# VikParuchuri/surya

Hardware: AMD Instinct MI355X
Metric: text-lines/sec recognised (whole node) (higher is better)
Workload: dtype bf16; 1 GPU; RecognitionPredictor device loop, 256 ragged 64x{128..512} crops/GPU, batch 256, max_tokens=48, REC-FULL synthetic weights (conditioned recipe, seed 0), tiles resident in HBM; parallelism=1 GPU, weights=conditioned

## Files before the change

surya_amd/csrc/attn_mfma.h:

```cpp
#pragma once
#include "common.h"
#include "kernels.h"

namespace sa {

typedef short s16x4 __attribute__((ext_vector_type(4)));

template <typename T, int D>
__global__ __launch_bounds__(128) void attn_mfma_kernel(const T* __restrict__ q, const T* __restrict__ k,
                                                        const T* __restrict__ v, T* __restrict__ out, AttnSegs sg,
                                                        long q_row, long q_head, long k_row, long k_head, long o_row, long o_head,
                                                        int group, int causal, float scale) {
    static_assert(D % 16 == 0 && D <= 128, "head dim");
    static_assert(sizeof(T) == 2, "16-bit storage types");
    constexpr int KC = 64;
    constexpr int PK = D + 8;
    constexpr int NKK = D / 16;
    constexpr int NDB = (D + 31) / 32;
    constexpr int CPR = D / 8;
    __shared__ __attribute__((aligned(16))) T ks[(KC + 1) * PK];
    __shared__ __attribute__((aligned(16))) T vs[(KC + 1) * PK];

    const int tile = blockIdx.x, head = blockIdx.y, kvh = head / group;
    const int seg = sg.tile_seg[tile], q0 = sg.tile_q0[tile], L = sg.seg_len[seg];
    const int tid = threadIdx.x, lane = tid & 63, wave = tid >> 6;
    const int ql = lane & 31, h = lane >> 5;
    const int qi = q0 + wave * 32 + ql;

    u32x4 qf[NKK];
    {
        const T* qp = q + sg.q_off[seg] + (long)min(qi, L - 1) * q_row + (long)head * q_head + h * 8;
#pragma unroll
        for (int kk = 0; kk < NKK; ++kk) qf[kk] = *reinterpret_cast<const u32x4*>(qp + kk * 16);
    }
    f32x16 oacc[NDB];
#pragma unroll
    for (int db = 0; db < NDB; ++db)
#pragma unroll
        for (int r = 0; r < 16; ++r) oacc[db][r] = 0.f;
    float mrun = -INFINITY, lrun = 0.f;
    const float sl2 = scale * 1.44269504088896340736f;

    const int kend = causal ? min(L, q0 + 64) : L;
    const T* kbase = k + sg.k_off[seg] + (long)kvh * k_head;
    const T* vbase = v + sg.v_off[seg] + (long)kvh * k_head;
    const int tr_off = ((lane & 15) >> 2) * PK + ((lane >> 4) & 1) * 16 + (lane & 3) * 4 + h * 4 * PK;

    constexpr int NST = KC * CPR / 128;
    static_assert(KC * CPR % 128 == 0, "staging split");
    u32x4 kreg[NST], vreg[NST];
    auto fetch = [&](int kc) {
        const int nk = min(KC, kend - kc);
#pragma unroll
// ... 48 lines not shown
        mrun = mnew;
        float psum = 0.f;
#pragma unroll
        for (int kb = 0; kb < 2; ++kb)
#pragma unroll
            for (int r = 0; r < 16; ++r) {
                const float pv = exp2f((sacc[kb][r] - mnew) * sl2);
                sacc[kb][r] = pv;
                psum += pv;
            }
        lrun = lrun * alpha + psum;
#pragma unroll
        for (int db = 0; db < NDB; ++db)
#pragma unroll
            for (int r = 0; r < 16; ++r) oacc[db][r] *= alpha;

#pragma unroll
        for (int t = 0; t < 4; ++t) {
            const int kb = t >> 1, o8 = (t & 1) * 8;
            u32x4 pf;
            pf[0] = H16<T>::pk(sacc[kb][o8 + 0], sacc[kb][o8 + 1]);
            pf[1] = H16<T>::pk(sacc[kb][o8 + 2], sacc[kb][o8 + 3]);
            pf[2] = H16<T>::pk(sacc[kb][o8 + 4], sacc[kb][o8 + 5]);
            pf[3] = H16<T>::pk(sacc[kb][o8 + 6], sacc[kb][o8 + 7]);
#pragma unroll
            for (int db = 0; db < NDB; ++db) {
                const T* vp = vs + t * 16 * PK + db * 32 + tr_off;
                const s16x4 lo = __builtin_amdgcn_ds_read_tr16_b64_v4i16((__attribute__((address_space(3))) s16x4*)(vp));
                const s16x4 hi = __builtin_amdgcn_ds_read_tr16_b64_v4i16((__attribute__((address_space(3))) s16x4*)(vp + 8 * PK));
                typedef short s16x8 __attribute__((ext_vector_type(8)));
                const s16x8 vf = __builtin_shufflevector(lo, hi, 0, 1, 2, 3, 4, 5, 6, 7);
                oacc[db] = H16<T>::mfma(vf, pf, oacc[db]);
            }
        }
        __syncthreads();
    }

    const float ltot = lrun + __shfl_xor(lrun, 32, 64);
    if (qi < L) {
        const float inv = 1.0f / ltot;
        T* op = out + sg.o_off[seg] + (long)qi * o_row + (long)head * o_head;
#pragma unroll
        for (int db = 0; db < NDB; ++db)
#pragma unroll
            for (int g = 0; g < 4; ++g) {
                const int d0 = db * 32 + g * 8 + h * 4;
                if (d0 < D) store4(op + d0, oacc[db][4 * g] * inv, oacc[db][4 * g + 1] * inv, oacc[db][4 * g + 2] * inv,
                                   oacc[db][4 * g + 3] * inv);
            }
    }
}

template <typename T>
int launch_attn(int D, const T* q, const T* k, const T* v, T* o, const AttnSegs& sg, int n_tiles, int heads, long q_row, long q_head,
                long k_row, long k_head, long o_row, long o_head, int group, int causal, float scale, hipStream_t s) {
    if (n_tiles <= 0) return SA_OK;
    auto go = [&](auto kern, int threads) {
        hipLaunchKernelGGL(kern, dim3(n_tiles, heads), dim3(threads), 0, s, q, k, v, o, sg, q_row, q_head, k_row, k_head, o_row, o_head, group,
                           causal, scale);
        return (int)hipGetLastError();
    };
    if constexpr (sizeof(T) == 2) {
        if (D == 32) return go(attn_mfma_kernel<T, 32>, 128);
        if (D == 64) return go(attn_mfma_kernel<T, 64>, 128);
        if (D == 80) return go(attn_mfma_kernel<T, 80>, 128);
        if (D == 128) return go(attn_mfma_kernel<T, 128>, 128);
    } else {
        static_assert(std::is_same<T, float>::value, "the VALU kernel is the fp32 reference-mode path only");
        if (D == 32) return go(attn_valu_kernel<T, 32>, 256);
        if (D == 64) return go(attn_valu_kernel<T, 64>, 256);
        if (D == 80) return go(attn_valu_kernel<T, 80>, 256);
        if (D == 128) return go(attn_valu_kernel<T, 128>, 256);
    }
    return SA_ERR_UNSUPPORTED;
}

}
```

surya_amd/csrc/common.h:

```cpp
#pragma once
#include <hip/hip_runtime.h>
#include <cstdlib>
#include <stdint.h>
#include <stdio.h>
#include <type_traits>

#include "../../include/surya_amd.h"

namespace sa {

typedef unsigned short bf16_t;
typedef __attribute__((ext_vector_type(4))) float f32x4;
typedef __attribute__((ext_vector_type(16))) float f32x16;
typedef __attribute__((ext_vector_type(8))) __bf16 bf16x8;
typedef unsigned int u32x4 __attribute__((ext_vector_type(4)));


#define SA_HIP(expr)                                                                                   \
    do {                                                                                               \
        hipError_t _e = (expr);                                                                        \
        if (_e != hipSuccess) {                                                                        \
            fprintf(stderr, "[surya_amd] %s:%d %s -> %s\n", __FILE__, __LINE__, #expr, hipGetErrorString(_e)); \
            return (int)_e;                                                                            \
        }                                                                                              \
// ... 208 lines not shown
    } else {
        return gelu_erf_f(x);
    }
}
__device__ __forceinline__ float gelu_tanh_f(float x) { return 0.5f * x * (1.0f + tanhf(0.7978845608028654f * (x + 0.044715f * x * x * x))); }
__device__ __forceinline__ float sigmoid_f(float x) { return 1.0f / (1.0f + __expf(-x)); }
__device__ __forceinline__ float hardswish_f(float x) {
    float t;
    asm("v_fma_f32 %0, %1, %2, 0.5 clamp" : "=v"(t) : "v"(x), "s"(1.0f / 6.0f));
    return x * t;
}
typedef float f32x2_hs __attribute__((ext_vector_type(2)));
__device__ __forceinline__ f32x2_hs hardswish_pk(f32x2_hs x) {
    f32x2_hs t;
    const f32x2_hs c = {1.0f / 6.0f, 1.0f / 6.0f};
    asm("v_pk_fma_f32 %0, %1, %2, 0.5 op_sel_hi:[1,0,0] clamp" : "=v"(t) : "v"(x), "s"(c));
    return x * t;
}

struct Tuning {
    int graph = 0;
    int split_target = 256;
    int split_min_kt = 4;
    int split_max = 8;
    int bigtile = 3;
    int bigtile_any = 0;
    int big_m_split = -1;
    int big_m_gateup = -1;
    int mx_big_m_split = -1;
    int mx_big_m_gateup = -1;
    int gateup_ring = 2;
    int dring = 1;
    int dring_min_kt = 0;
    int conv_persist = 3;
    int dwconv_pipe = 2;
    int conv_lean = 1;
    int bigtile_ratio_pct = 0;
    int bigtile_min_k = 0;
    int glds = 2;
    int dattn = 4;
    int rnorm = 2;
    int ghead = 2;
    int fuse_embed = 1;
    int kvprefetch = 0;
    int lmhead = 1;
    int dattn_db = 0;
    int lay_ln = 1;
    int det_head_blk = 1;
    int det_fuse = 1023;
    int det_up4 = 1;
    int fmb_chunk = 64;
    int persist = 1;
    int ocrerr_cls_only = 1;
};
inline Tuning& tuning() { static Tuning t; return t; }
inline int& tuning_epoch() { static int e = 0; return e; }

inline void poison_arena(void* p, size_t bytes) {
    static const bool on = [] { const char* e = getenv("SURYA_AMD_POISON"); return e && e[0] == '1'; }();
    if (on) { (void)hipMemset(p, 0xFF, bytes); (void)hipDeviceSynchronize(); }
}

struct AttrOnce {
    size_t granted[64] = {};
    template <typename F> void ensure(F kern, size_t lds) {
        int dev = 0;
        (void)hipGetDevice(&dev);
        size_t& g = granted[dev & 63];
        if (lds > g || g == 0) {
            (void)hipFuncSetAttribute(reinterpret_cast<const void*>(kern), hipFuncAttributeMaxDynamicSharedMemorySize, (int)lds);
            g = lds > g ? lds : g;
            if (g == 0) g = 1;
        }
    }
};

constexpr int SA_ALT_NONE = 0x7fffffff;
__device__ __forceinline__ bool alt_after(float v, int c, float pv, int pc) { return (v < pv) | ((v == pv) & (c > pc)); }
__device__ __forceinline__ bool alt_before(float v, int c, float bv, int bc) { return (v > bv) | ((v == bv) & (c < bc)); }
__device__ __forceinline__ float2 alt_next(const float2* cand, int n, float pv, int pc) {
    float cb = -INFINITY;
    int ci = SA_ALT_NONE;
    for (int k = 0; k < n; ++k) {
        const float v = cand[k].x;
        const int cc = __float_as_int(cand[k].y);
        const bool take = (v > -INFINITY) & alt_after(v, cc, pv, pc) & alt_before(v, cc, cb, ci);
        cb = take ? v : cb;
        ci = take ? cc : ci;
    }
    return make_float2(cb, __int_as_float(ci));
}

static inline int cdiv(int a, int b) { return (a + b - 1) / b; }
static inline long cdivl(long a, long b) { return (a + b - 1) / b; }

}
```

surya_amd/csrc/rec_engine.h:

```cpp
#pragma once
#include <algorithm>
#include <cstdlib>
#include <cstring>
#include <initializer_list>
#include <map>
#include <memory>
#include <set>
#include <vector>

#include "../../include/surya_amd.h"
#include "gemm.h"
#include "gemm_mx.h"
#include "kernels.h"
#include "decode_attn.h"
#include "decode_attn_kv8.h"
#include "attn_mfma.h"
#include "beam.h"
#include "lexicon.h"
#include "boost.h"

namespace sa {

struct Stager {
    char* host = nullptr;
// ... 564 lines not shown
                    return rc;
                if ((rc = rmsnorm(ex, He, WE(l, SA_RE_NORM2), eh, He, nullptr, Pi, He, c.enc_eps, s))) return rc;
                if ((rc = gemm<EPI_SWIGLU>(eh, He, WE(l, SA_RE_GU_W), He, emlp, c.enc_inter_pad, WE(l, SA_RE_GU_B), nullptr, 0,
                                           Pi, 2 * c.enc_inter_pad, He, s))) return rc;
                if ((rc = gemm<EPI_RESIDUAL>(emlp, c.enc_inter_pad, WE(l, SA_RE_DOWN_W), c.enc_inter_pad, ex, He,
                                             WE(l, SA_RE_DOWN_B), ex, He, Pi, He, c.enc_inter_pad, s))) return rc;
            }
            if ((rc = rmsnorm(ex, He, W(SA_RW_MERGER_LN), eh, He, nullptr, Pi, He, 1e-6f, s))) return rc;
            const int Mg = Pi / unit, Hm = He * unit;
            if ((rc = gemm<EPI_GELU>(eh, Hm, W(SA_RW_FC1_W), Hm, emh, Hm, W(SA_RW_FC1_B), nullptr, 0, Mg, Hm, Hm, s))) return rc;
            if ((rc = gemm<EPI_BIAS>(emh, Hm, W(SA_RW_FC2_W), Hm, emerged, c.enc_out_hidden, W(SA_RW_FC2_B), nullptr, 0, Mg,
                                     c.enc_out_hidden, Hm, s))) return rc;
            if ((rc = launch_scatter_image<T>(emerged, W(SA_RW_IMG_H), W(SA_RW_IMG_W), d_dst, d_hidx, d_widx, dst, Mg, c.dec_hidden, s))) return rc;
            patch_base += P;
            tok_base += P / unit;
            i0 = i1;
        }
        return SA_OK;
    }

    int encode_only(const float* tiles, const int32_t* grid_hw, int n, void* out, hipStream_t s) override {
        if (c.enc_out_hidden != c.dec_hidden) return SA_ERR_SHAPE;
        long ntok = 0;
        for (int i = 0; i < n; ++i) ntok += (long)grid_hw[2 * i] * grid_hw[2 * i + 1] / (c.merge * c.merge);
        std::vector<int> ident(ntok);
        for (long i = 0; i < ntok; ++i) ident[i] = (int)i;
        return encode(tiles, grid_hw, n, ident, reinterpret_cast<T*>(out), s);
    }

    int encode_ahead(const float* tiles, const int32_t* grid_hw, int n, hipStream_t s) override {
        if (c.enc_out_hidden != c.dec_hidden) return SA_ERR_SHAPE;
        if (n == 0) {
            ahead_consumed = ahead_tokens = 0;
            return SA_OK;
        }
        if (n < 0 || !tiles || !grid_hw) return SA_ERR_ARG;
        if (ahead_consumed != ahead_tokens) return SA_ERR_STATE;
        long ntok = 0;
        for (int i = 0; i < n; ++i) ntok += (long)grid_hw[2 * i] * grid_hw[2 * i + 1] / (c.merge * c.merge);
        if (ntok > std::max(c.max_prefill_tokens, c.max_slots)) return SA_ERR_SHAPE;
        std::vector<int> ident(ntok);
        for (long i = 0; i < ntok; ++i) ident[i] = (int)i;
        SA_HIP(hipEventRecord(ev_ahead_in, s));
        SA_HIP(hipStreamWaitEvent(estream, ev_ahead_in, 0));
        if (ahead_free_recorded) SA_HIP(hipStreamWaitEvent(estream, ev_ahead_free, 0));
        int rc = encode(tiles, grid_hw, n, ident, emb_ahead, estream, st_enc);
        if (rc) return rc;
        SA_HIP(hipEventRecord(ev_ahead_done, estream));
        ahead_tokens = ntok;
        ahead_consumed = 0;
        return SA_OK;
    }

    int decoder_layers_prefill(int M, const int* d_tok_slot, const int* d_tok_pos, const AttnSegs* sg, int n_tiles, hipStream_t s) {
        const int Hd = c.dec_hidden, nq = c.dec_heads, nkv = c.dec_kv_heads, d = c.dec_head_dim, I = c.dec_inter;
        const int qkv_d = (nq + 2 * nkv) * d;
        const float scale = 1.0f / sqrtf((float)d);
        const size_t layer_kv = (size_t)c.max_slots * nkv * c.max_kv_len * d;
        const float* inv_freq = reinterpret_cast<const float*>(w[SA_RW_DEC_INVFREQ]);
        int rc;
        for (int l = 0; l < c.dec_layers; ++l) {
            T* kc = kcache + l * layer_kv;
            T* vc = vcache + l * layer_kv;
            if ((rc = rmsnorm(dx, Hd, WD(l, SA_RD_LN1), dh, Hd, nullptr, M, Hd, c.dec_eps, s))) return rc;
            if ((rc = gemm<EPI_BIAS>(dh, Hd, WD(l, SA_RD_QKV_W), Hd, dqkv, qkv_d, WD(l, SA_RD_QKV_B), nullptr, 0, M, qkv_d, Hd, s)))
                return rc;
            if ((rc = launch_rope_kv_append<T>(dqkv, d_tok_slot, d_tok_pos, rope_cs, kc, vc, M, nq, nkv, d, c.max_kv_len, s))) return rc;
            if constexpr (std::is_same<T, bf16_t>::value) {
                if (kv8) {
                    const size_t l8 = (size_t)c.max_slots * nkv, T8 = tmax8();
                    if ((rc = launch_kv8_quant_rows(d, kc, vc, d_tok_slot, d_tok_pos, M, k8c + l * l8 * c.max_kv_len * d, v8tc + l * l8 * d * T8,
                                                    ksc8 + l * l8 * T8, vsc8 + l * l8 * T8, nkv, c.max_kv_len, s))) return rc;
                }
            }
            if ((rc = launch_attn<T>(d, dqkv, kc, vc, dattn, *sg, n_tiles, nq, qkv_d, d, d, (long)c.max_kv_len * d, (long)nq * d, d,
                                     nq / nkv, 1, scale, s))) return rc;
            if ((rc = gemm<EPI_RESIDUAL>(dattn, (long)nq * d, WD(l, SA_RD_O_W), (long)nq * d, dx, Hd, nullptr, dx, Hd, M, Hd, nq * d,
                                         s))) return rc;
            if ((rc = rmsnorm(dx, Hd, WD(l, SA_RD_LN2), dh, Hd, nullptr, M, Hd, c.dec_eps, s))) return rc;
            if ((rc = gemm<EPI_SWIGLU>(dh, Hd, WD(l, SA_RD_GU_W), Hd, dmlp, I, nullptr, nullptr, 0, M, 2 * I, Hd, s))) return rc;
            if ((rc = gemm<EPI_RESIDUAL>(dmlp, I, WD(l, SA_RD_DOWN_W), I, dx, Hd, nullptr, dx, Hd, M, Hd, I, s))) return rc;
        }
        return SA_OK;
    }

    struct Half { int r0, M; float* part; hipStream_t s; };

    int splitk_gemm(const T* X, long ldx, const T* Wt, long ldw, int M, int N, int K, float* part_, int* S, hipStream_t s) {
        GemmArgs<T, T> a{X, ldx, Wt, ldw, nullptr, 0, nullptr, nullptr, 0, M, N, K, 1, part_};
        int rc = launch_gemm_splitk<T>(a, s);
        *S = a.splitk;
        return rc;
    }
    int reduce_residual_norm(int S, int M, const float* part_, T* x, const T* wnorm, T* y, hipStream_t s, uint8_t* y8 = nullptr,
                             uint8_t* sy = nullptr, const T* pf_cache = nullptr, const Half* h = nullptr) {
        KvPrefetch pf;
        if (pf_cache && h && tuning().kvprefetch && (c.dec_head_dim * sizeof(T)) % 16 == 0) {
            pf.base = reinterpret_cast<const unsigned char*>(pf_cache);
            pf.slots = active_dev + h->r0; pf.lens = row_len + h->r0;
            pf.head_stride = (long)c.max_kv_len * c.dec_head_dim * sizeof(T);
            pf.slot_stride = pf.head_stride * c.dec_kv_heads;
            pf.heads = c.dec_kv_heads; pf.row_bytes = c.dec_head_dim * (int)sizeof(T); pf.max_rows = c.max_kv_len;
        }
        return launch_reduce_norm<T>(part_, S, M, x, wnorm, y, c.dec_hidden, c.dec_eps, y8, sy, c.max_slots, pf, s);
    }
    int splitk_gemm_mx(const uint8_t* X, const uint8_t* SX, long ldx, const uint8_t* Wq, const uint8_t* SW, int M, int N, int K,
                       float* part_, int* S, hipStream_t s) {
        MxArgs a{X, ldx, SX, Wq, (long)K, SW, M, N, K, (long)c.max_slots, (long)N};
        a.part = part_;
        int rc = launch_gemm_mx_splitk(a, s);
        *S = a.splitk;
        return rc;
    }

    void drop_graphs() {
        for (auto& kv : graphs) (void)hipGraphExecDestroy(kv.second);
        graphs.clear(); seen_keys.clear();
    }
    int set_kv_fp8(int on) override {
        if constexpr (!std::is_same<T, bf16_t>::value) return on ? SA_ERR_UNSUPPORTED : SA_OK;
        if (on && excluded(M_KV8)) return SA_ERR_STATE;
        if ((on != 0) != kv8) drop_graphs();
        if (!on) { kv8 = false; return SA_OK; }
        const int d = c.dec_head_dim;
        if (d != 128 && d != 64 && d != 32) return SA_ERR_UNSUPPORTED;
        if (c.dec_heads / c.dec_kv_heads > 8) return SA_ERR_UNSUPPORTED;
        if (!kv8_arena.dev) {
            const size_t rows = (size_t)c.dec_layers * c.max_slots * c.dec_kv_heads, T8 = tmax8();
            Carve cv;
// ... 610 lines not shown
        int rc, S = 1;
        const bool q8 = mx();
        const int A = nq * d;
        uint8_t *hh8 = nullptr, *shh = nullptr, *at8 = nullptr, *sat = nullptr, *ml8 = nullptr, *sml = nullptr;
        if (q8) {
            hh8 = dh8 + (size_t)h.r0 * Hd; shh = sdh + (size_t)h.r0 * 4;
            at8 = dattn8 + (size_t)h.r0 * A; sat = sattn + (size_t)h.r0 * 4;
            ml8 = dmlp8 + (size_t)h.r0 * I; sml = smlp + (size_t)h.r0 * 4;
        }
        rc = -1;
        if constexpr (MX_OK) {
            if (q8) rc = splitk_gemm_mx(hh8, shh, Hd, MXW(l, SA_MX_QKV_W), MXW(l, SA_MX_QKV_S), M, qkv_d, Hd, h.part, &S, s);
        }
        if (!q8) rc = splitk_gemm(hh, Hd, WD(l, SA_RD_QKV_W), Hd, M, qkv_d, Hd, h.part, &S, s);
        if (rc) return rc;
        bool launched = false;
        if constexpr (std::is_same<T, bf16_t>::value) {
            if (kv8) {
                const size_t l8 = (size_t)c.max_slots * nkv, T8 = tmax8();
                DecodeAttnKv8Args a{h.part, S, WD(l, SA_RD_QKV_B), at, k8c + l * l8 * c.max_kv_len * d, v8tc + l * l8 * d * T8, ksc8 + l * l8 * T8,
                                    vsc8 + l * l8 * T8, act, rl, rope_cs, M, nq, nkv, d, c.max_kv_len, scale, at8, sat, c.max_slots};
                if ((rc = launch_decode_attn_kv8(a, s))) return rc;
                launched = true;
            }
        }
        if (!launched) {
            DecodeAttnArgs<T> a{h.part, S, WD(l, SA_RD_QKV_B), at, kc, vc, act, rl, rope_cs, M, nq, nkv, d, c.max_kv_len, scale, ctx_bound, at8, sat,
                                c.max_slots};
            if ((rc = launch_decode_attn<T>(a, s))) return rc;
        }
        const bool last = (l + 1 == c.dec_layers);
        const T* wnext = last ? W(SA_RW_DEC_NORM) : WD(l + 1, SA_RD_LN1);
        T* ynext = last ? dlast + (size_t)h.r0 * Hd : hh;
        if constexpr (MX_OK) if (q8) {
            if ((rc = splitk_gemm_mx(at8, sat, A, MXW(l, SA_MX_O_W), MXW(l, SA_MX_O_S), M, Hd, A, h.part, &S, s))) return rc;
            if ((rc = reduce_residual_norm(S, M, h.part, x, WD(l, SA_RD_LN2), hh, s, hh8, shh))) return rc;
            MxArgs g{hh8, Hd, shh, MXW(l, SA_MX_GU_W), Hd, MXW(l, SA_MX_GU_S), M, 2 * I, Hd, (long)c.max_slots, (long)2 * I};
            g.Q = ml8; g.ldq = I; g.SQ = sml; g.sq_rows = c.max_slots;
            if ((rc = launch_gemm_mx<MX_EPI_SWIGLU>(g, s))) return rc;
            if ((rc = splitk_gemm_mx(ml8, sml, I, MXW(l, SA_MX_DOWN_W), MXW(l, SA_MX_DOWN_S), M, Hd, I, h.part, &S, s))) return rc;
            return reduce_residual_norm(S, M, h.part, x, wnext, ynext, s, last ? dlast8 + (size_t)h.r0 * Hd : hh8,
                                        last ? slast + (size_t)h.r0 * 4 : shh);
        }
        const bool warm = !last && !kv8;
        const T* v_next = warm ? vcache + (size_t)(l + 1) * layer_kv : nullptr;
        const T* k_next = warm ? kcache + (size_t)(l + 1) * layer_kv : nullptr;
        if ((rc = splitk_gemm(at, (long)nq * d, WD(l, SA_RD_O_W), (long)nq * d, M, Hd, nq * d, h.part, &S, s))) return rc;
        if ((rc = reduce_residual_norm(S, M, h.part, x, WD(l, SA_RD_LN2), hh, s, nullptr, nullptr, v_next, &h))) return rc;
        if ((rc = gemm<EPI_SWIGLU>(hh, Hd, WD(l, SA_RD_GU_W), Hd, ml, I, nullptr, nullptr, 0, M, 2 * I, Hd, s))) return rc;
        if ((rc = splitk_gemm(ml, I, WD(l, SA_RD_DOWN_W), I, M, Hd, I, h.part, &S, s))) return rc;
        return reduce_residual_norm(S, M, h.part, x, wnext, ynext, s, nullptr, nullptr, k_next, &h);
    }

    int heads(int rows, const int* d_last_row, const int* d_row_slot, int step, int len_inc, bool normed, hipStream_t s, bool fuse_next = false) {
        const int Hd = c.dec_hidden;
        int rc;
        T* last = dlast;
        float4* am = amax;
        if (!normed && (rc = rmsnorm(dx, Hd, W(SA_RW_DEC_NORM), last, Hd, d_last_row, rows, Hd, c.dec_eps, s))) return rc;
        int bn_used = 0;
        auto lm_head = [&](auto& a, auto&& launch) -> int {
            a.amax = am;
            if (forcing) {
                a.forced = forced_cols(d_row_slot);
            } else {
                if (n_token_masks > 0) a.tmask = token_mask(d_row_slot);
                if (topk()) a.alt = alt_part;
            }
            const int rc_ =forcing ? launch(a, HeadEpi<0>{}) : topk() ? launch(a, HeadEpi<1>{}) : n_token_masks > 0 ? launch(a, HeadEpi<2>{}) : launch(a, HeadEpi<3>{});
            bn_used = a.bn_used;
            if (rc_ || bst_states == 0) return rc_;
            a.amax = amax_b;
            a.tmask = TokenMask{};
            const int rc_b = launch(a, HeadEpi<3>{});
            return rc_b ? rc_b : a.bn_used != bn_used ? (int)SA_ERR_STATE : (int)SA_OK;
        };
        if (mx() && normed) {
            if constexpr (std::is_same<T, bf16_t>::value) {
                static constexpr int EPIS[4] = {MX_EPI_FORCED, MX_EPI_TOPK, MX_EPI_ARGMAX_MASK, MX_EPI_ARGMAX};
                MxArgs a{dlast8, Hd, slast, MXG(SA_MX_LM_W), Hd, MXG(SA_MX_LM_S), rows, c.vocab, Hd, (long)c.max_slots, (long)c.vocab};
                a.bias = W(SA_RW_LM_B);
                if ((rc = lm_head(a, [&](MxArgs& a_, auto e) { return launch_gemm_mx<EPIS[decltype(e)::value]>(a_, s); }))) return rc;
            }
        } else {
            static constexpr int EPIS[4] = {EPI_FORCED, EPI_TOPK, EPI_ARGMAX_MASK, EPI_ARGMAX};
            GemmArgs<T, float> a{last, Hd, W(SA_RW_LM_W), Hd, logits, c.vocab, W(SA_RW_LM_B), nullptr, 0, rows, c.vocab, Hd};
            if ((rc = lm_head(a, [&](GemmArgs<T, float>& a_, auto e) { return launch_gemm<T, float, EPIS[decltype(e)::value]>(a_, s); }))) return rc;
        }
        const int tiles_n = cdiv(c.vocab, bn_used);
        const size_t so = (size_t)step * c.max_slots;
        last_rows = rows;
        last_heads_mx = mx() && normed;
        float2* bt = topk() ? best_tot : nullptr;
        ForcedHead fh;
        if (forcing) fh = ForcedHead{forced_table, forced_cursor, flogit, SA_MAX_FORCED_TOKENS, greedy_token + so, greedy_prob + so, forced_logprob + so};
        auto combine = [&]() -> int {
            if ((rc = (int)hipGetLastError()) || !topk()) return rc;
            hipLaunchKernelGGL(topk_combine_kernel, dim3(rows), dim3(SA_ALT_THREADS), 0, s, alt_part, tiles_n, d_row_slot, bt,
                               alt_token + so * SA_MAX_ALTERNATIVES, alt_prob + so * SA_MAX_ALTERNATIVES);
            return (int)hipGetLastError();
        };
        const bool fz = fuse_next;
        HeadArgs<T> ha{reinterpret_cast<const float4*>(am), tiles_n, rows, last, Hd, W(SA_RW_BBOX_W), W(SA_RW_BBOX_B), d_row_slot, c.eos_token_id,
                       c.pad_token_id, (float)c.bbox_size, out_token + so, out_score + so, out_bbox + so * 6, next_token, kv_len, len_inc};
        ha.table = fz ? W(SA_RW_TOK_EMBED) : (const T*)nullptr;
        ha.wnorm = WD(0, SA_RD_LN1); ha.x = dx; ha.y = dh; ha.row_len = row_len; ha.Tmax = c.max_kv_len; ha.eps = c.dec_eps;
        ha.y8 = (fz && mx()) ? dh8 : (uint8_t*)nullptr; ha.sy = (fz && mx()) ? sdh : (uint8_t*)nullptr; ha.srows = c.max_slots;
        ha.best_tot = bt; ha.fh = fh;
        if (pat_states > 0)
            ha.ph = PatternHead{pat_tok_class, pat_next_state, pat_state_mask, SA_MAX_PATTERN_CLASSES, c.vocab, slot_state, slot_mask};
        if (bst_states > 0) {
            BoostHeadArgs<T> bh{ha, reinterpret_cast<const float4*>(amax_b), slot_bst_beta, plain_token + so, plain_prob + so};
// ... 24 lines not shown
            for (int t = 0; t < L; ++t) {
                const int id = input_ids[a + t];
                if (id < 0 || id >= c.vocab) return SA_ERR_ARG;
                const bool img = (id == c.image_token_id);
                ids[a + t] = img ? -1 : id;
                if (img) img_pos.push_back(a + t);
                tok_slot[a + t] = slot_ids[i]; tok_pos[a + t] = t;
            }
            sg.seg_len.push_back(L);
            sg.q_off.push_back((long)a * (nq + 2 * nkv) * d);
            sg.k_off.push_back((long)slot_ids[i] * nkv * c.max_kv_len * d);
            sg.v_off.push_back((long)slot_ids[i] * nkv * c.max_kv_len * d);
            sg.o_off.push_back((long)a * nq * d);
            sg.add_tiles(i, L);
        }
        long ntok = 0;
        for (int i = 0; i < n_images; ++i) ntok += (long)grid_hw[2 * i] * grid_hw[2 * i + 1] / (c.merge * c.merge);
        if ((long)img_pos.size() != ntok) return SA_ERR_SHAPE;
        int rc;
        st_small.begin();
        const int* d_slots = st_small.put(slot_ids, n_seqs);
        const int* d_lens = st_small.put(lens);
        const int* d_last = st_small.put(last_row);
        if (!d_last) return SA_ERR_NOMEM;
        if ((rc = st_small.flush(s))) return rc;
        {
            st.begin();
            const int* d_ids = st.put(ids);
            if (!d_ids) return SA_ERR_NOMEM;
            if ((rc = st.flush(s))) return rc;
            if ((rc = launch_embed_tokens<T>(W(SA_RW_TOK_EMBED), d_ids, dx, Ttot, c.dec_hidden, s))) return rc;
        }
        if (n_images > 0 && tiles) {
            if ((rc = encode(tiles, grid_hw, n_images, img_pos, dx, s))) return rc;
        } else if (n_images > 0) {
            if (ahead_consumed + ntok > ahead_tokens) return SA_ERR_STATE;
            st.begin();
            const int* d_img = st.put(img_pos);
            if (!d_img) return SA_ERR_NOMEM;
            if ((rc = st.flush(s))) return rc;
            SA_HIP(hipStreamWaitEvent(s, ev_ahead_done, 0));
            if ((rc = launch_scatter_rows<T>(emb_ahead + ahead_consumed * c.dec_hidden, d_img, dx, (int)ntok, c.dec_hidden, s))) return rc;
            ahead_consumed += ntok;
            SA_HIP(hipEventRecord(ev_ahead_free, s));
            ahead_free_recorded = true;
        }
        st.begin();
        const int* d_tok_slot = st.put(tok_slot);
        const int* d_tok_pos = st.put(tok_pos);
        AttnSegs d_sg = stage_segs(st, sg);
        if (!d_sg.o_off) return SA_ERR_NOMEM;
        if ((rc = st.flush(s))) return rc;
        hipLaunchKernelGGL(set_slot_state_kernel, dim3(cdiv(n_seqs, 256)), dim3(256), 0, s, d_slots, d_lens, kv_len, n_seqs);
        if ((rc = decoder_layers_prefill(Ttot, d_tok_slot, d_tok_pos, &d_sg, (int)sg.tile_seg.size(), s))) return rc;
        if ((rc = heads(n_seqs, d_last, d_slots, 0, 0, false, s)) || beam == 0) return rc;
        return beam_step(d_slots, 1, n_seqs, 0, 1, s);
    }

    int set_active(const int32_t* slots, int n, hipStream_t s) override {
        if (n < 0 || n > c.max_slots) return SA_ERR_ARG;
        n_active = n;
        for (int i = 0; i < n; ++i)
            if (slots[i] < 0 || slots[i] >= c.max_slots) return SA_ERR_ARG;
        if (beam > 0) {
            if (n % beam) return SA_ERR_ARG;
            for (int i = 0; i < n; ++i) {
                const int lead = slots[i - i % beam];
                if (lead % beam || slots[i] != lead + i % beam || (i >= beam && i % beam == 0 && lead <= slots[i - beam])) return SA_ERR_ARG;
            }
        }
        h_active.assign(slots, slots + n);
        if (n == 0) return SA_OK;
        st_small.begin();
        const int* d = st_small.put(slots, n);
        if (!d) return SA_ERR_NOMEM;
        int rc = st_small.flush(s);
        if (rc) return rc;
        SA_HIP(hipMemcpyAsync(active_dev, d, n * sizeof(int), hipMemcpyDeviceToDevice, s));
        return SA_OK;
    }

    bool can_fuse_embed() const {
        return tuning().fuse_embed && head2_ok() && c.dec_hidden <= 2 * 4 * SA_HEAD_THREADS && cdiv(c.vocab, 320) <= 4 * SA_HEAD_THREADS &&
               cdiv(c.vocab, 64) <= 4 * SA_HEAD_THREADS;
    }
    int decode_eager(int M, int n_steps, int step0, hipStream_t s) {
        int rc;
        const Half h{0, M, part, s};
        const bool fuse = can_fuse_embed() && beam == 0;
        if (h_len.size() < (size_t)c.max_slots) h_len.resize(c.max_slots, 0);
        for (int step = 0; step < n_steps; ++step) {
            ctx_bound = 0;
            for (int a : h_active) {
                ctx_bound = std::max(ctx_bound, h_len[a] + 1);
                h_len[a] = std::min(h_len[a] + 1, c.max_kv_len);
            }
            if ((step == 0 || !fuse) && (rc = decode_embed(h))) return rc;
            for (int l = 0; l < c.dec_layers; ++l)
                if ((rc = decode_layer(l, h))) return rc;
            if ((rc = heads(M, nullptr, active_dev, step0 + step, 1, true, s, fuse && step + 1 < n_steps))) return rc;
            if (beam > 0 && (rc = beam_step(active_dev, beam, M / beam, step0 + step, 0, s))) return rc;
        }
        return SA_OK;
    }

    int decode(int n_steps, hipStream_t s) override { return decode_steps(n_steps, 0, s); }

    int decode_async(int n_steps, int ring, hipStream_t s) override {
// ... 93 lines not shown
```

surya_amd/csrc/rec_model.hip:

```cpp
#include "rec_engine.h"
#include "rec_ops.h"
#include "rec_prep.h"

namespace sa {

template <int D, int MAXG>
static int decode_attn_flash(const DecodeAttnArgs<bf16_t>& a, hipStream_t s) {
    const Tuning& t = tuning();
    if (t.dattn == 3) return decode_attn_as<decode_attn_flash_kernel<D, MAXG>>(a, decode_attn_flash_lds<D, MAXG>(), s, a.out8, a.sout, a.srows);
    if (t.dattn_db == 1 || (t.dattn_db == 0 && !t.graph && a.ctx_bound > 128 && a.rows * a.nkv <= 256))
        return decode_attn_as<decode_attn_flash2_kernel<D, MAXG, true>>(a, decode_attn_flash2_lds<D, MAXG, true>(), s, a.out8, a.sout, a.srows);
    return decode_attn_as<decode_attn_flash2_kernel<D, MAXG, false>>(a, decode_attn_flash2_lds<D, MAXG, false>(), s, a.out8, a.sout, a.srows);
}
template <typename T>
int launch_decode_attn(const DecodeAttnArgs<T>& a, hipStream_t s) {
    const int G = a.nq / a.nkv, d = a.d;
    if constexpr (std::is_same<T, bf16_t>::value) {
        if (d == 128 && G <= 5) return decode_attn_flash<128, 5>(a, s);
        if (d == 128 && G <= 8) return decode_attn_flash<128, 8>(a, s);
        if (d == 64 && G <= 8) return decode_attn_flash<64, 8>(a, s);
        if (d == 32 && G <= 8) return decode_attn_flash<32, 8>(a, s);
    }
    if (a.out8) return SA_ERR_UNSUPPORTED;
    if (d == 128 && G <= 5) return decode_attn_as<decode_attn_mfma_kernel<T, 128, 5>>(a, decode_attn_mfma_lds<T, 128, 5>(), s);
// ... 502 lines not shown
    if (!X || !W || !part || !splitk) return SA_ERR_ARG;
    GemmArgs<bf16_t, bf16_t> a{reinterpret_cast<const bf16_t*>(X), ldx, reinterpret_cast<const bf16_t*>(W), ldw, nullptr, 0, nullptr, nullptr, 0, M, N, K, 1, part};
    const int rc = launch_gemm_splitk<bf16_t>(a, (hipStream_t)stream);
    *splitk = a.splitk;
    return rc;
}

int surya_op_gemm_mx(int mode, const uint8_t* X, const uint8_t* SX, const uint8_t* W, const uint8_t* SW, int M, int N, int K,
                     float* C, int* splitk, uint8_t* q_out, uint8_t* sq_out, void* stream) {
    if (!X || !SX || !W || !SW) return SA_ERR_ARG;
    MxArgs a{X, (long)K, SX, W, (long)K, SW, M, N, K, (long)M, (long)N};
    hipStream_t s = (hipStream_t)stream;
    if (mode == 0) {
        if (!C) return SA_ERR_ARG;
        a.C = C; a.ldc = N;
        return launch_gemm_mx<MX_EPI_F32>(a, s);
    }
    if (mode == 1) {
        if (!C || !splitk) return SA_ERR_ARG;
        a.part = C;
        int rc = launch_gemm_mx_splitk(a, s);
        *splitk = a.splitk;
        return rc;
    }
    if (mode == 2) {
        if (!q_out || !sq_out) return SA_ERR_ARG;
        a.Q = q_out; a.ldq = N / 2; a.SQ = sq_out; a.sq_rows = M;
        return launch_gemm_mx<MX_EPI_SWIGLU>(a, s);
    }
    return SA_ERR_ARG;
}

int surya_rec_preprocess(const uint8_t* pages, const void* lines, int n_lines, uint8_t* mask_arena, float* mid_arena, float* tiles,
                         int patch_size, int merge_size, float pad_value, const float* mean, const float* std, int any_poly,
                         int max_stage1_width, int pixel_stride, void* stream) {
    if (!pages || !lines || !tiles || !mean || !std || n_lines < 0 || patch_size <= 0 || merge_size <= 0) return SA_ERR_ARG;
    if (pixel_stride != 3 && pixel_stride != 4) return SA_ERR_ARG;
    sa::prep::PrepArgs p;
    p.pages = pages; p.lines = reinterpret_cast<const sa::prep::LineDesc*>(lines); p.n_lines = n_lines;
    p.mask = mask_arena; p.mid = mid_arena; p.tiles = tiles; p.ps = patch_size; p.merge = merge_size; p.pad = pad_value;
    for (int i = 0; i < 3; ++i) { p.mean[i] = mean[i]; p.std[i] = std[i]; }
    p.max_mid_w = max_stage1_width;
    p.pix = pixel_stride;
    return sa::prep::prep_run(p, any_poly, max_stage1_width > 0, (hipStream_t)stream);
}

int surya_set_tuning(const char* key, int value) {
    if (!key) return SA_ERR_ARG;
    Tuning& t = tuning();
    struct { const char* k; int* v; } tab[] = {
        {"graph", &t.graph}, {"split_target", &t.split_target}, {"split_min_kt", &t.split_min_kt}, {"split_max", &t.split_max},
        {"bigtile", &t.bigtile}, {"bigtile_any", &t.bigtile_any}, {"conv_lean", &t.conv_lean}, {"conv_persist", &t.conv_persist}, {"dwconv_pipe", &t.dwconv_pipe}, {"bigtile_ratio_pct", &t.bigtile_ratio_pct}, {"gateup_ring", &t.gateup_ring}, {"dring", &t.dring}, {"dring_min_kt", &t.dring_min_kt}, {"big_m_split", &t.big_m_split}, {"big_m_gateup", &t.big_m_gateup}, {"mx_big_m_split", &t.mx_big_m_split}, {"mx_big_m_gateup", &t.mx_big_m_gateup}, {"glds", &t.glds}, {"bigtile_min_k", &t.bigtile_min_k}, {"dattn", &t.dattn}, {"rnorm", &t.rnorm},
        {"ghead", &t.ghead}, {"fuse_embed", &t.fuse_embed}, {"persist", &t.persist}, {"lmhead", &t.lmhead}, {"kvprefetch", &t.kvprefetch},
        {"dattn_db", &t.dattn_db}, {"lay_ln", &t.lay_ln}, {"det_head_blk", &t.det_head_blk}, {"det_fuse", &t.det_fuse}, {"det_up4", &t.det_up4}, {"fmb_chunk", &t.fmb_chunk}, {"ocrerr_cls_only", &t.ocrerr_cls_only}};
    for (auto& e : tab)
        if (!strcmp(e.k, key)) {
            if (*e.v != value) ++tuning_epoch();
            *e.v = value;
            return SA_OK;
        }
    return SA_ERR_ARG;
}

int surya_gemm_ring_status(int reset) {
    const int a = sa::ring_error(reset != 0), b = sa::rec_f16_ring_error(reset != 0);
    return a ? a : b;
}

int surya_prof_enable(int on) {
    GemmProfiler& pf = gemm_profiler();
    if (on) pf.start(); else pf.enabled = false;
    return SA_OK;
}

__global__ void prof_null_kernel() {}

int surya_prof_event_overhead(void* stream, double* ms) {
    if (!ms) return SA_ERR_ARG;
    hipStream_t s = (hipStream_t)stream;
    constexpr int N = 201;
    hipEvent_t ev[2 * N];
    for (auto& e : ev) SA_HIP(hipEventCreate(&e));
    for (int i = 0; i < 32; ++i) hipLaunchKernelGGL(prof_null_kernel, dim3(1), dim3(64), 0, s);
    for (int i = 0; i < N; ++i) {
        SA_HIP(hipEventRecord(ev[2 * i], s));
        hipLaunchKernelGGL(prof_null_kernel, dim3(1), dim3(64), 0, s);
        SA_HIP(hipEventRecord(ev[2 * i + 1], s));
    }
    SA_HIP(hipStreamSynchronize(s));
    std::vector<float> t(N);
    for (int i = 0; i < N; ++i) SA_HIP(hipEventElapsedTime(&t[i], ev[2 * i], ev[2 * i + 1]));
    for (auto& e : ev) (void)hipEventDestroy(e);
    std::sort(t.begin(), t.end());
    *ms = t[N / 2];
    return SA_OK;
}

int surya_prof_read2(int max_cfg, int* launches, double* ms, double* flops, double* bytes, double* slab_bytes) {
    GemmProfiler& pf = gemm_profiler();
    if (!launches || !ms || !flops || !bytes || max_cfg < GemmProfiler::NCFG) return SA_ERR_ARG;
    SA_HIP(hipDeviceSynchronize());
    const int ncfg = std::min(max_cfg, (int)GemmProfiler::NCFG_ALL);
    for (int c = 0; c < ncfg; ++c) { launches[c] = 0; ms[c] = flops[c] = bytes[c] = 0.0; if (slab_bytes) slab_bytes[c] = 0.0; }
    for (int i = 0; i < pf.n; ++i) {
        const int c = pf.cfg_of[i];
        if (c >= ncfg) continue;
        float t = 0.f;
// ... 109 lines not shown
```

Measured before the change: 3150 lines/s.

## Add persistent 4-head vision attention kernel and trim last prefill layer to final rows

After: 3189 lines/s, median of 6. +1.2%, better.

```diff
diff --git a/surya_amd/csrc/attn_mfma.h b/surya_amd/csrc/attn_mfma.h
--- a/surya_amd/csrc/attn_mfma.h
+++ b/surya_amd/csrc/attn_mfma.h
@@ -1,4 +1,6 @@
 #pragma once
+#include <algorithm>
+
 #include "common.h"
 #include "kernels.h"
 
@@ -153,6 +155,190 @@
 }
 
 template <typename T>
+__global__ __launch_bounds__(512) void attn_lines_kernel(const T* __restrict__ q, const T* __restrict__ k, const T* __restrict__ v,
+                                                         T* __restrict__ out, AttnSegs sg, long q_row, long k_row, long o_row, int n_tiles,
+                                                         int n_groups, float scale) {
+    static_assert(sizeof(T) == 2, "16-bit storage types");
+    constexpr int D = 80, HG = 4, KC = 64, PK = D + 8, NKK = D / 16, NDB = (D + 31) / 32, CPR = D / 8;
+    constexpr int RUN = HG * CPR;
+    constexpr int HB = (KC + 1) * PK;
+    extern __shared__ __attribute__((aligned(16))) unsigned char attn_lines_lds[];
+    T* const ks_all = reinterpret_cast<T*>(attn_lines_lds);
+    T* const vs_all = ks_all + HG * HB;
+
+    const int tid = threadIdx.x, lane = tid & 63, wave = tid >> 6;
+    const int hs = wave >> 1, ql = lane & 31, h = lane >> 5;
+    const T* const ks = ks_all + hs * HB;
+    const T* const vs = vs_all + hs * HB;
+    const float sl2 = scale * 1.44269504088896340736f;
+    const int tr_off = ((lane & 15) >> 2) * PK + ((lane >> 4) & 1) * 16 + (lane & 3) * 4 + h * 4 * PK;
+
+    struct Item { int qi, L; const T *qp, *kb, *vb; T* op; };
+    auto item = [&](int w) {
+        const int tile = w / n_groups, hg = w % n_groups;
+        const int seg = sg.tile_seg[tile];
+        Item it;
+        it.L = sg.seg_len[seg];
+        it.qi = sg.tile_q0[tile] + (wave & 1) * 32 + ql;
+        it.qp = q + sg.q_off[seg] + (long)min(it.qi, it.L - 1) * q_row + (long)(hg * HG + hs) * D + h * 8;
+        it.kb = k + sg.k_off[seg] + (long)hg * (HG * D);
+        it.vb = v + sg.v_off[seg] + (long)hg * (HG * D);
+        it.op = out + sg.o_off[seg] + (long)it.qi * o_row + (long)(hg * HG + hs) * D;
+        return it;
+    };
+
+    constexpr int NST = KC * RUN / 512;
+    static_assert(KC * RUN % 512 == 0, "staging split");
+    u32x4 qf[NKK], kreg[NST], vreg[NST];
+    auto fetch_q = [&](const Item& it) {
+#pragma unroll
+        for (int kk = 0; kk < NKK; ++kk) qf[kk] = *reinterpret_cast<const u32x4*>(it.qp + kk * 16);
+    };
+    auto fetch = [&](const T* base, u32x4* reg, int kc, int kend) {
+        const int nk = min(KC, kend - kc);
+#pragma unroll
+        for (int it = 0; it < NST; ++it) {
+            const int c = tid + it * 512, r = min(c / RUN, nk - 1), p = c % RUN;
+            reg[it] = *reinterpret_cast<const u32x4*>(base + (long)(kc + r) * k_row + p * 8);
+        }
+    };
+    auto stage = [&](T* img, const u32x4* reg, int nk) {
+#pragma unroll
+        for (int it = 0; it < NST; ++it) {
+            const int c = tid + it * 512, r = c / RUN, p = c % RUN;
+            const u32x4 z = {0u, 0u, 0u, 0u};
+            *reinterpret_cast<u32x4*>(img + (p / CPR) * HB + r * PK + (p % CPR) * 8) = r < nk ? reg[it] : z;
+        }
+    };
+    const int n_work = n_tiles * n_groups;
+    int w = blockIdx.x;
+    Item cur = item(w);
+    fetch_q(cur);
+    fetch(cur.kb, kreg, 0, cur.L);
+    fetch(cur.vb, vreg, 0, cur.L);
+    for (; w < n_work; w += gridDim.x) {
+        const bool has_next = w + (int)gridDim.x < n_work;
+        const Item nxt = item(has_next ? w + (int)gridDim.x : w);
+        const int kend = cur.L;
+        f32x16 oacc[NDB];
+#pragma unroll
+        for (int db = 0; db < NDB; ++db)
+#pragma unroll
+            for (int r = 0; r < 16; ++r) oacc[db][r] = 0.f;
+        float mrun = -INFINITY, lrun = 0.f;
+        for (int kc = 0; kc < kend; kc += KC) {
+            const int nk = min(KC, kend - kc);
+            const bool last = kc + KC >= kend;
+            stage(ks_all, kreg, nk);
+            stage(vs_all, vreg, nk);
+            __syncthreads();
+            if (!last) {
+                fetch(cur.kb, kreg, kc + KC, kend);
+                fetch(cur.vb, vreg, kc + KC, kend);
+            } else if (has_next) {
+                fetch(nxt.kb, kreg, 0, nxt.L);
+                fetch(nxt.vb, vreg, 0, nxt.L);
+            }
+
+            f32x16 sacc[2];
+#pragma unroll
+            for (int kb = 0; kb < 2; ++kb) {
+#pragma unroll
+                for (int r = 0; r < 16; ++r) sacc[kb][r] = 0.f;
+                const T* kp = ks + (kb * 32 + ql) * PK + h * 8;
+#pragma unroll
+                for (int kk = 0; kk < NKK; ++kk) {
+                    const u32x4 kf = *reinterpret_cast<const u32x4*>(kp + kk * 16);
+                    sacc[kb] = H16<T>::mfma(kf, qf[kk], sacc[kb]);
+                }
+            }
+            if (last && has_next) fetch_q(nxt);
+            float bm = -INFINITY;
+#pragma unroll
+            for (int kb = 0; kb < 2; ++kb)
+#pragma unroll
+                for (int g = 0; g < 4; ++g)
+#pragma unroll
+                    for (int r = 0; r < 4; ++r) {
+                        const int j = kb * 32 + g * 8 + h * 4 + r;
+                        const float sv = (j < nk) ? sacc[kb][4 * g + r] : -INFINITY;
+                        sacc[kb][4 * g + r] = sv;
+                        bm = fmaxf(bm, sv);
+                    }
+            bm = fmaxf(bm, __shfl_xor(bm, 32, 64));
+            const float mnew = fmaxf(mrun, bm);
+            const float alpha = exp2f((mrun - mnew) * sl2);
+            mrun = mnew;
+            float psum = 0.f;
+#pragma unroll
+            for (int kb = 0; kb < 2; ++kb)
+#pragma unroll
+                for (int r = 0; r < 16; ++r) {
+                    const float pv = exp2f((sacc[kb][r] - mnew) * sl2);
+                    sacc[kb][r] = pv;
+                    psum += pv;
+                }
+            lrun = lrun * alpha + psum;
+#pragma unroll
+            for (int db = 0; db < NDB; ++db)
+#pragma unroll
+                for (int r = 0; r < 16; ++r) oacc[db][r] *= alpha;
+
+#pragma unroll
+            for (int t = 0; t < 4; ++t) {
+                const int kb = t >> 1, o8 = (t & 1) * 8;
+                u32x4 pf;
+                pf[0] = H16<T>::pk(sacc[kb][o8 + 0], sacc[kb][o8 + 1]);
+                pf[1] = H16<T>::pk(sacc[kb][o8 + 2], sacc[kb][o8 + 3]);
+                pf[2] = H16<T>::pk(sacc[kb][o8 + 4], sacc[kb][o8 + 5]);
+                pf[3] = H16<T>::pk(sacc[kb][o8 + 6], sacc[kb][o8 + 7]);
+#pragma unroll
+                for (int db = 0; db < NDB; ++db) {
+                    const T* vp = vs + t * 16 * PK + db * 32 + tr_off;
+                    const s16x4 lo = __builtin_amdgcn_ds_read_tr16_b64_v4i16((__attribute__((address_space(3))) s16x4*)(vp));
+                    const s16x4 hi = __builtin_amdgcn_ds_read_tr16_b64_v4i16((__attribute__((address_space(3))) s16x4*)(vp + 8 * PK));
+                    typedef short s16x8 __attribute__((ext_vector_type(8)));
+                    const s16x8 vf = __builtin_shufflevector(lo, hi, 0, 1, 2, 3, 4, 5, 6, 7);
+                    oacc[db] = H16<T>::mfma(vf, pf, oacc[db]);
+                }
+            }
+            __syncthreads();
+        }
+
+        const float ltot = lrun + __shfl_xor(lrun, 32, 64);
+        if (cur.qi < cur.L) {
+            const float inv = 1.0f / ltot;
+#pragma unroll
+            for (int db = 0; db < NDB; ++db)
+#pragma unroll
+                for (int g = 0; g < 4; ++g) {
+                    const int d0 = db * 32 + g * 8 + h * 4;
+                    if (d0 < D) store4(cur.op + d0, oacc[db][4 * g] * inv, oacc[db][4 * g + 1] * inv, oacc[db][4 * g + 2] * inv,
+                                       oacc[db][4 * g + 3] * inv);
+                }
+        }
+        cur = nxt;
+    }
+}
+
+template <typename T>
+int launch_attn_lines(const T* q, const T* k, const T* v, T* o, const AttnSegs& sg, int n_tiles, int heads, long q_row, long k_row, long o_row,
+                      float scale, hipStream_t s) {
+    constexpr size_t lds = (size_t)2 * 4 * 65 * 88 * sizeof(T);
+    static AttrOnce attr;
+    attr.ensure(attn_lines_kernel<T>, lds);
+    static int n_cu_of[64] = {};
+    int dev = 0;
+    (void)hipGetDevice(&dev);
+    int& n_cu = n_cu_of[dev & 63];
+    if (!n_cu && (hipDeviceGetAttribute(&n_cu, hipDeviceAttributeMultiprocessorCount, dev) != hipSuccess || n_cu <= 0)) n_cu = 256;
+    const long n_work = (long)n_tiles * (heads / 4);
+    hipLaunchKernelGGL(attn_lines_kernel<T>, dim3((unsigned)std::min<long>(n_work, n_cu)), dim3(512), lds, s, q, k, v, o, sg, q_row, k_row,
+                       o_row, n_tiles, heads / 4, scale);
+    return (int)hipGetLastError();
+}
+
+template <typename T>
 int launch_attn(int D, const T* q, const T* k, const T* v, T* o, const AttnSegs& sg, int n_tiles, int heads, long q_row, long q_head,
                 long k_row, long k_head, long o_row, long o_head, int group, int causal, float scale, hipStream_t s) {
     if (n_tiles <= 0) return SA_OK;
@@ -162,6 +348,11 @@
         return (int)hipGetLastError();
     };
     if constexpr (sizeof(T) == 2) {
+        if (D == 80 && tuning().vattn && heads % 4 == 0 && group == 1 && !causal && q_head == D && k_head == D && o_head == D && q_row == k_row &&
+            q_row % 64 == 0 && (reinterpret_cast<uintptr_t>(k) - reinterpret_cast<uintptr_t>(q)) % 128 == 0 &&
+            (reinterpret_cast<uintptr_t>(v) - reinterpret_cast<uintptr_t>(q)) % 128 == 0) {
+            return launch_attn_lines<T>(q, k, v, o, sg, n_tiles, heads, q_row, k_row, o_row, scale, s);
+        }
         if (D == 32) return go(attn_mfma_kernel<T, 32>, 128);
         if (D == 64) return go(attn_mfma_kernel<T, 64>, 128);
         if (D == 80) return go(attn_mfma_kernel<T, 80>, 128);
diff --git a/surya_amd/csrc/common.h b/surya_amd/csrc/common.h
--- a/surya_amd/csrc/common.h
+++ b/surya_amd/csrc/common.h
@@ -284,6 +284,8 @@
     int fmb_chunk = 64;
     int persist = 1;
     int ocrerr_cls_only = 1;
+    int vattn = 1;
+    int prefill_trim = 1;
 };
 inline Tuning& tuning() { static Tuning t; return t; }
 inline int& tuning_epoch() { static int e = 0; return e; }
diff --git a/surya_amd/csrc/rec_engine.h b/surya_amd/csrc/rec_engine.h
--- a/surya_amd/csrc/rec_engine.h
+++ b/surya_amd/csrc/rec_engine.h
@@ -640,7 +640,9 @@
         return SA_OK;
     }
 
-    int decoder_layers_prefill(int M, const int* d_tok_slot, const int* d_tok_pos, const AttnSegs* sg, int n_tiles, hipStream_t s) {
+    int decoder_layers_prefill(int M, const int* d_tok_slot, const int* d_tok_pos, const AttnSegs* sg, int n_tiles, const int* d_last_row,
+                               int n_seqs, const T** x_last, hipStream_t s) {
+        *x_last = nullptr;
         const int Hd = c.dec_hidden, nq = c.dec_heads, nkv = c.dec_kv_heads, d = c.dec_head_dim, I = c.dec_inter;
         const int qkv_d = (nq + 2 * nkv) * d;
         const float scale = 1.0f / sqrtf((float)d);
@@ -663,6 +665,18 @@
             }
             if ((rc = launch_attn<T>(d, dqkv, kc, vc, dattn, *sg, n_tiles, nq, qkv_d, d, d, (long)c.max_kv_len * d, (long)nq * d, d,
                                      nq / nkv, 1, scale, s))) return rc;
+            if (l == c.dec_layers - 1 && tuning().prefill_trim && n_seqs < M) {
+                T *ca = dqkv, *cx = dh, *ch = dx;
+                if ((rc = launch_embed_tokens<T>(dattn, d_last_row, ca, n_seqs, nq * d, s))) return rc;
+                if ((rc = launch_embed_tokens<T>(dx, d_last_row, cx, n_seqs, Hd, s))) return rc;
+                if ((rc = gemm<EPI_RESIDUAL>(ca, (long)nq * d, WD(l, SA_RD_O_W), (long)nq * d, cx, Hd, nullptr, cx, Hd, n_seqs, Hd, nq * d,
+                                             s))) return rc;
+                if ((rc = rmsnorm(cx, Hd, WD(l, SA_RD_LN2), ch, Hd, nullptr, n_seqs, Hd, c.dec_eps, s))) return rc;
+                if ((rc = gemm<EPI_SWIGLU>(ch, Hd, WD(l, SA_RD_GU_W), Hd, dmlp, I, nullptr, nullptr, 0, n_seqs, 2 * I, Hd, s))) return rc;
+                if ((rc = gemm<EPI_RESIDUAL>(dmlp, I, WD(l, SA_RD_DOWN_W), I, cx, Hd, nullptr, cx, Hd, n_seqs, Hd, I, s))) return rc;
+                *x_last = cx;
+                return SA_OK;
+            }
             if ((rc = gemm<EPI_RESIDUAL>(dattn, (long)nq * d, WD(l, SA_RD_O_W), (long)nq * d, dx, Hd, nullptr, dx, Hd, M, Hd, nq * d,
                                          s))) return rc;
             if ((rc = rmsnorm(dx, Hd, WD(l, SA_RD_LN2), dh, Hd, nullptr, M, Hd, c.dec_eps, s))) return rc;
@@ -1379,12 +1393,13 @@
         return reduce_residual_norm(S, M, h.part, x, wnext, ynext, s, nullptr, nullptr, k_next, &h);
     }
 
-    int heads(int rows, const int* d_last_row, const int* d_row_slot, int step, int len_inc, bool normed, hipStream_t s, bool fuse_next = false) {
+    int heads(int rows, const int* d_last_row, const int* d_row_slot, int step, int len_inc, bool normed, hipStream_t s, bool fuse_next = false,
+              const T* x_rows = nullptr) {
         const int Hd = c.dec_hidden;
         int rc;
         T* last = dlast;
         float4* am = amax;
-        if (!normed && (rc = rmsnorm(dx, Hd, W(SA_RW_DEC_NORM), last, Hd, d_last_row, rows, Hd, c.dec_eps, s))) return rc;
+        if (!normed && (rc = rmsnorm(x_rows ? x_rows : dx, Hd, W(SA_RW_DEC_NORM), last, Hd, x_rows ? nullptr : d_last_row, rows, Hd, c.dec_eps, s))) return rc;
         int bn_used = 0;
         auto lm_head = [&](auto& a, auto&& launch) -> int {
             a.amax = am;
@@ -1515,8 +1530,9 @@
         if (!d_sg.o_off) return SA_ERR_NOMEM;
         if ((rc = st.flush(s))) return rc;
         hipLaunchKernelGGL(set_slot_state_kernel, dim3(cdiv(n_seqs, 256)), dim3(256), 0, s, d_slots, d_lens, kv_len, n_seqs);
-        if ((rc = decoder_layers_prefill(Ttot, d_tok_slot, d_tok_pos, &d_sg, (int)sg.tile_seg.size(), s))) return rc;
-        if ((rc = heads(n_seqs, d_last, d_slots, 0, 0, false, s)) || beam == 0) return rc;
+        const T* x_last = nullptr;
+        if ((rc = decoder_layers_prefill(Ttot, d_tok_slot, d_tok_pos, &d_sg, (int)sg.tile_seg.size(), d_last, n_seqs, &x_last, s))) return rc;
+        if ((rc = heads(n_seqs, d_last, d_slots, 0, 0, false, s, false, x_last)) || beam == 0) return rc;
         return beam_step(d_slots, 1, n_seqs, 0, 1, s);
     }
 
diff --git a/surya_amd/csrc/rec_model.hip b/surya_amd/csrc/rec_model.hip
--- a/surya_amd/csrc/rec_model.hip
+++ b/surya_amd/csrc/rec_model.hip
@@ -578,7 +578,8 @@
         {"graph", &t.graph}, {"split_target", &t.split_target}, {"split_min_kt", &t.split_min_kt}, {"split_max", &t.split_max},
         {"bigtile", &t.bigtile}, {"bigtile_any", &t.bigtile_any}, {"conv_lean", &t.conv_lean}, {"conv_persist", &t.conv_persist}, {"dwconv_pipe", &t.dwconv_pipe}, {"bigtile_ratio_pct", &t.bigtile_ratio_pct}, {"gateup_ring", &t.gateup_ring}, {"dring", &t.dring}, {"dring_min_kt", &t.dring_min_kt}, {"big_m_split", &t.big_m_split}, {"big_m_gateup", &t.big_m_gateup}, {"mx_big_m_split", &t.mx_big_m_split}, {"mx_big_m_gateup", &t.mx_big_m_gateup}, {"glds", &t.glds}, {"bigtile_min_k", &t.bigtile_min_k}, {"dattn", &t.dattn}, {"rnorm", &t.rnorm},
         {"ghead", &t.ghead}, {"fuse_embed", &t.fuse_embed}, {"persist", &t.persist}, {"lmhead", &t.lmhead}, {"kvprefetch", &t.kvprefetch},
-        {"dattn_db", &t.dattn_db}, {"lay_ln", &t.lay_ln}, {"det_head_blk", &t.det_head_blk}, {"det_fuse", &t.det_fuse}, {"det_up4", &t.det_up4}, {"fmb_chunk", &t.fmb_chunk}, {"ocrerr_cls_only", &t.ocrerr_cls_only}};
+        {"dattn_db", &t.dattn_db}, {"lay_ln", &t.lay_ln}, {"det_head_blk", &t.det_head_blk}, {"det_fuse", &t.det_fuse}, {"det_up4", &t.det_up4}, {"fmb_chunk", &t.fmb_chunk}, {"ocrerr_cls_only", &t.ocrerr_cls_only},
+        {"vattn", &t.vattn}, {"prefill_trim", &t.prefill_trim}};
     for (auto& e : tab)
         if (!strcmp(e.k, key)) {
             if (*e.v != value) ++tuning_epoch();
```
